# cmavro/GNN-RAG

Measured on AMD Instinct MI355X. Metric: kg_edges_aggregated_per_sec, higher is better.
Workload: dtype f32

## Files before the change

gnn-rag_amd/csrc/tables_b3.hip:

```cpp
#include "gnnrag_common.h"
#include "dense_internal.h"

namespace gnnrag {

#ifndef GNNRAG_TAB_TPW
#define GNNRAG_TAB_TPW 3
#endif
#ifndef GNNRAG_TAB_MINBLK
#define GNNRAG_TAB_MINBLK 2
#endif
constexpr int kTabTPW = GNNRAG_TAB_TPW;
constexpr int kTabNTH = 7;
constexpr int kTabNKB = 7;
constexpr int kTabSlots = 26;
constexpr int kTabQBytes = 160 * 1024 - 3 * kTabNTH * 16 * kTabSlots * 16 - 64;

struct TabArgs {
  const float* T[2];
  const float* ins;
  const float* W;
  float* P;
  const int2* rows;
  int32_t M, D, I, ldw;
  int32_t ct0;
  int32_t npass;
};

__device__ __forceinline__ int opaque_i(int x) {
  asm volatile("" : "+v"(x));
  return x;
}

template <int CTRL, int BANK>
__device__ __forceinline__ float dpp_b3(float old, float x) {
  return __int_as_float(__builtin_amdgcn_update_dpp(__float_as_int(old), __float_as_int(x), CTRL, 0xf, BANK, false));
}
__device__ __forceinline__ float row16_sum4_b3(const float (&v)[4], int lane) {
  const bool b0 = lane & 1, b1 = lane & 2;
  float w2[2];
#pragma unroll
  for (int j = 0; j < 2; ++j) {
    const float send = b0 ? v[j] : v[j + 2];
    w2[j] = (b0 ? v[j + 2] : v[j]) + dpp_b3<0xB1, 0xf>(send, send);
  }
  const float send = b1 ? w2[0] : w2[1];
  float w = (b1 ? w2[1] : w2[0]) + dpp_b3<0x4E, 0xf>(send, send);
  const float t4 = dpp_b3<0x104, 0x5>(w, w);
  w += dpp_b3<0x114, 0xA>(t4, w);
  w += dpp_b3<0x128, 0xf>(w, w);
  return w;
}

__device__ __forceinline__ int tab_lds_row(int j) {
  if (j < 64) return ((j & 3) << 4) + (j >> 2);
  return j;
}

__device__ __forceinline__ constexpr int tab_stage_rows(int ctn) { return ctn < kTabNTH ? ctn * 16 + 1 : ctn * 16; }

template <int CTN, bool QLDS>
__device__ __forceinline__ void tables_b3_part(const TabArgs& a, unsigned char* lds, int col0, int bmin, int nq) {
  constexpr int RB = kTabSlots * 16;
  constexpr int PL = kTabNTH * 16 * RB;
  constexpr int ctn = CTN;
  const int tid = threadIdx.x, lane = tid & 63, wave = tid >> 6;
  const int fr = lane & 15, fg = lane >> 4;
  const int d = blockIdx.y;
  const int D = a.D, I = a.I;
  const int ncol = min(ctn * 16, D - col0);
  const float* T = a.T[d];
  float* P = a.P + (size_t)d * a.M * D;
  const f32x4 zero4 = {0.f, 0.f, 0.f, 0.f};
  constexpr int NKB = kTabNKB;
  const int KC = D >> 2;

  const long long U = ((long long)a.M + 15) >> 4;
  const int c0 = (int)(U * blockIdx.x / gridDim.x), c1 = (int)(U * (blockIdx.x + 1) / gridDim.x);
  const int nchunk = c1 - c0;
  const int w0 = c0 + (int)((long long)nchunk * wave / 8), w1 = c0 + (int)((long long)nchunk * (wave + 1) / 8);

  if (tid < 16) reinterpret_cast<unsigned*>(lds + 3 * PL)[tid] = 0u;
  float* qarea = reinterpret_cast<float*>(lds + 3 * PL + 64);
  constexpr bool q_in_lds = QLDS;
  if (q_in_lds) {
    const float* src = a.ins + (size_t)bmin * I * D;
    for (int x = tid * 4; x < nq * I * D; x += 512 * 4)
      *reinterpret_cast<f32x4*>(qarea + x) = *reinterpret_cast<const f32x4*>(src + x);
  }

  for (int pass = 0; pass < a.npass; ++pass) {
    const int tbase = w0 + pass * kTabTPW;
    const int ntile = max(0, min(kTabTPW, w1 - tbase));
    f32x4 acc[kTabTPW][CTN];
#pragma unroll
    for (int j = 0; j < kTabTPW; ++j)
#pragma unroll
      for (int nt = 0; nt < CTN; ++nt) acc[j][nt] = zero4;

    for (int i = 0; i < I; ++i) {
      __syncthreads();
      {
        const int wcol = (1 + 2 * i + d) * D;
        const int total = tab_stage_rows(ctn) * kTabSlots * 2;
        constexpr int UN = 6;
        for (int base = 0; base < total; base += 512 * UN) {
          f32x4 v[UN];
          int off[UN];
#pragma unroll
          for (int u = 0; u < UN; ++u) {
            const int idx = base + u * 512 + tid;
            const int j = idx / (kTabSlots * 2), kc = idx - j * (kTabSlots * 2);
            v[u] = zero4;
            off[u] = idx < total ? tab_lds_row(j) * RB + kc * 8 : -1;
            if (idx < total && j < ncol && kc < KC)
              v[u] = *reinterpret_cast<const f32x4*>(a.W + (size_t)(col0 + j) * a.ldw + wcol + 4 * kc);
          }
#pragma unroll
          for (int u = 0; u < UN; ++u) {
            if (off[u] >= 0) {
              const Split3 sp = split3(v[u]);
              unsigned char* dst = lds + off[u];
              *reinterpret_cast<uint2*>(dst) = sp.hi;
              *reinterpret_cast<uint2*>(dst + PL) = sp.mid;
              *reinterpret_cast<uint2*>(dst + 2 * PL) = sp.lo;
            }
          }
        }
      }
      __syncthreads();

      int toff[kTabTPW], qoff[kTabTPW];
#pragma unroll
      for (int j = 0; j < kTabTPW; ++j) {
        const int m = min((tbase + (j < ntile ? j : 0)) * 16 + fr, a.M - 1);
        const int2 br = a.rows[m];
        toff[j] = br.y * D + 8 * fg;
        qoff[j] = ((br.x - bmin) * I + i) * D + 8 * fg;
      }
      const int kmax = D - 8;
      f32x4 traw[kTabTPW][2];
#pragma unroll
      for (int j = 0; j < kTabTPW; ++j) {
        const float* tp = T + toff[j] + (min(8 * fg, kmax) - 8 * fg);
        traw[j][0] = *reinterpret_cast<const f32x4*>(tp);
        traw[j][1] = *reinterpret_cast<const f32x4*>(tp + 4);
      }
      for (int kb = 0; kb < NKB; ++kb) {
        const bool kok = 32 * kb + 8 * fg <= kmax;
        const int kbn = min(kb + 1, NKB - 1);
        const int kon = min(32 * kbn + 8 * fg, kmax) - 8 * fg;
        const int koq = min(32 * kb + 8 * fg, kmax) - 8 * fg;
        const unsigned char* wb = lds + fr * RB + kb * 64 + fg * 16;
#pragma unroll
        for (int j = 0; j < kTabTPW; ++j) {
          if (j < ntile) {
            const f32x4 t0 = traw[j][0], t1 = traw[j][1];
            {
              const float* tp = T + toff[j] + kon;
              traw[j][0] = *reinterpret_cast<const f32x4*>(tp);
              traw[j][1] = *reinterpret_cast<const f32x4*>(tp + 4);
            }
            __builtin_amdgcn_sched_barrier(0);
            f32x4 q0, q1;
            if constexpr (QLDS) {
              const float* qp = qarea + qoff[j] + koq;
              q0 = *reinterpret_cast<const f32x4*>(qp);
              q1 = *reinterpret_cast<const f32x4*>(qp + 4);
            } else {
              const float* qp = a.ins + (size_t)bmin * I * D + qoff[j] + koq;
              q0 = *reinterpret_cast<const f32x4*>(qp);
              q1 = *reinterpret_cast<const f32x4*>(qp + 4);
            }
            const Split3 s0 = split3(kok ? __builtin_elementwise_max(t0 * q0, zero4) : zero4);
            const Split3 s1 = split3(kok ? __builtin_elementwise_max(t1 * q1, zero4) : zero4);
            typedef unsigned u32x4 __attribute__((ext_vector_type(4)));
            bf16x8 ap[3];
            ap[0] = __builtin_bit_cast(bf16x8, (u32x4){s0.hi.x, s0.hi.y, s1.hi.x, s1.hi.y});
            ap[1] = __builtin_bit_cast(bf16x8, (u32x4){s0.mid.x, s0.mid.y, s1.mid.x, s1.mid.y});
            ap[2] = __builtin_bit_cast(bf16x8, (u32x4){s0.lo.x, s0.lo.y, s1.lo.x, s1.lo.y});
            constexpr int PA[6] = {1, 2, 0, 1, 0, 0};
            constexpr int PB[6] = {1, 0, 2, 0, 1, 0};
#pragma unroll
            for (int nt = 0; nt < CTN; nt += 2) {
              bf16x8 b0[3], b1[3];
#pragma unroll
              for (int pl = 0; pl < 3; ++pl) {
                b0[pl] = __builtin_bit_cast(bf16x8, *reinterpret_cast<const f32x4*>(wb + pl * PL + nt * 16 * RB));
                b1[pl] = b0[pl];
                if (nt + 1 < CTN)
                  b1[pl] = __builtin_bit_cast(bf16x8, *reinterpret_cast<const f32x4*>(wb + pl * PL + (nt + 1) * 16 * RB));
              }
#pragma unroll
              for (int p = 0; p < 6; ++p) {
                acc[j][nt] = __builtin_amdgcn_mfma_f32_16x16x32_bf16(ap[PA[p]], b0[PB[p]], acc[j][nt], 0, 0, 0);
                if (nt + 1 < CTN)
                  acc[j][nt + 1] = __builtin_amdgcn_mfma_f32_16x16x32_bf16(ap[PA[p]], b1[PB[p]], acc[j][nt + 1], 0, 0, 0);
              }
            }
          }
        }
      }
    }

#pragma unroll
    for (int j = 0; j < kTabTPW; ++j) {
      if (j < ntile) {
        const int rbase = (tbase + j) * 16 + 4 * fg;
#pragma unroll
        for (int q = 0; q < 4; ++q) {
          const int row = rbase + q;
          if (row < a.M) {
            float* prow = P + (size_t)row * D + col0;
            static_assert(CTN >= 4, "a column part holds at least the interleaved group");
            {
              const f32x4 v = {acc[j][0][q], acc[j][1][q], acc[j][2][q], acc[j][3][q]};
              const int c = 4 * fr;
              if (c + 4 <= ncol) *reinterpret_cast<f32x4*>(prow + c) = v;
              else {
#pragma unroll
                for (int e = 0; e < 4; ++e)
                  if (c + e < ncol) prow[c + e] = v[e];
              }
            }
#pragma unroll
            for (int nt = 4; nt < CTN; ++nt) {
              const int c = nt * 16 + fr;
              if (c < ncol) prow[c] = acc[j][nt][q];
            }
          }
        }
      }
    }
  }
}

__global__ __launch_bounds__(512, GNNRAG_TAB_MINBLK) void k_tables_b3(TabArgs a) {
  extern __shared__ __attribute__((aligned(16))) unsigned char lds[];
  const int NT = (a.D + 15) >> 4;
  const int h = blockIdx.z;
  const int ctn = h == 0 ? a.ct0 : NT - a.ct0;
  const int col0 = h == 0 ? 0 : a.ct0 * 16;
  const long long U = ((long long)a.M + 15) >> 4;
  const int c0 = (int)(U * blockIdx.x / gridDim.x), c1 = (int)(U * (blockIdx.x + 1) / gridDim.x);
  const int rlo = min(c0 * 16, a.M - 1), rhi = min(c1 * 16, a.M) - 1;
  const int bmin = a.rows[rlo].x, bmax = a.rows[max(rhi, rlo)].x;
  const int nq = bmax - bmin + 1;
  const bool q_in_lds = (size_t)nq * a.I * a.D * sizeof(float) <= kTabQBytes;
#define GNNRAG_TAB_CASE(N)                                                  \
  case N:                                                                   \
    if (q_in_lds) tables_b3_part<N, true>(a, lds, col0, bmin, nq);          \
    else tables_b3_part<N, false>(a, lds, col0, bmin, nq);                  \
    break;
  switch (ctn) {
    GNNRAG_TAB_CASE(6) GNNRAG_TAB_CASE(7)
    default: break;
  }
#undef GNNRAG_TAB_CASE
}

constexpr int kVqHalf = 32 * kTabNKB;
constexpr int kVqRowB = 2 * kVqHalf * 2;
#ifndef GNNRAG_VQ_TPW
#define GNNRAG_VQ_TPW 5
#endif
#ifndef GNNRAG_VQ_UN
#define GNNRAG_VQ_UN 3
#endif
constexpr int kVqTPW = GNNRAG_VQ_TPW;

struct VqArgs {
  const unsigned char* planes;
  const float* ins;
  const float* W;
  float* P;
  const int2* rows;
  const int* rel_off;
  int32_t M, D, I, ldw, R1;
  int32_t ct0;
  int32_t nchunk;
  int32_t dir0;
  float* zero;
  int64_t zero_n;
};

template <int CTN, int UN>
__device__ __forceinline__ void vq_stage(const VqArgs& a, unsigned char* lds, const float* qarea, int col0, int ncol,
                                         int d, int s) {
  constexpr int RB = kTabSlots * 16;
  constexpr int PL = kTabNTH * 16 * RB;
  const int tid = threadIdx.x;
  const int D = a.D, I = a.I, KC = D >> 2;
  const f32x4 zero4 = {0.f, 0.f, 0.f, 0.f};
  const int total = tab_stage_rows(CTN) * kTabSlots * 2;
  for (int base = 0; base < total; base += 512 * UN) {
    f32x4 v[UN];
#pragma unroll
    for (int u = 0; u < UN; ++u) v[u] = zero4;
    for (int i = 0; i < I; ++i) {
      f32x4 w[UN];
      const float* wsrc = a.W + (size_t)col0 * a.ldw + (1 + 2 * i + d) * D;
#pragma unroll
      for (int u = 0; u < UN; ++u) {
        const int idx = base + u * 512 + tid;
        const int j = idx / (kTabSlots * 2), kc = idx - j * (kTabSlots * 2);
        w[u] = *reinterpret_cast<const f32x4*>(wsrc + (size_t)min(j, ncol - 1) * a.ldw + 4 * min(kc, KC - 1));
      }
#pragma unroll
      for (int u = 0; u < UN; ++u) {
        const int idx = base + u * 512 + tid;
        const int kc = idx % (kTabSlots * 2);
        f32x4 q = *reinterpret_cast<const f32x4*>(qarea + i * D + 4 * min(kc, KC - 1));
        q = __builtin_elementwise_max(s ? -q : q, zero4);
        v[u] += w[u] * q;
      }
    }
#pragma unroll
    for (int u = 0; u < UN; ++u) {
      const int idx = base + u * 512 + tid;
      const int j = idx / (kTabSlots * 2), kc = idx - j * (kTabSlots * 2);
      if (idx < total) {
        const Split3 sp = split3(j < ncol && kc < KC ? v[u] : zero4);
        unsigned char* dst = lds + tab_lds_row(j) * RB + kc * 8;
        *reinterpret_cast<uint2*>(dst) = sp.hi;
        *reinterpret_cast<uint2*>(dst + PL) = sp.mid;
        *reinterpret_cast<uint2*>(dst + 2 * PL) = sp.lo;
      }
    }
  }
}

template <int CTN>
__device__ __forceinline__ void tables_vq_part(const VqArgs& a, unsigned char* lds, int col0) {
  constexpr int RB = kTabSlots * 16;
  constexpr int PL = kTabNTH * 16 * RB;
  constexpr int NKB = kTabNKB;
  const int tid = threadIdx.x, lane = tid & 63, wave = tid >> 6;
  const int fr = lane & 15, fg = lane >> 4;
  const int d = a.dir0 + blockIdx.y;
  const int g = blockIdx.x / a.nchunk, ch = blockIdx.x - g * a.nchunk;
  const int D = a.D, I = a.I;
  const int r0 = a.rel_off[g], r1 = a.rel_off[g + 1];
  if (r1 <= r0) return;
  const int ncol = min(CTN * 16, D - col0);
  const int KC = D >> 2;
  const f32x4 zero4 = {0.f, 0.f, 0.f, 0.f};
  float* P = a.P + (size_t)d * a.M * D;
  const unsigned char* planes = a.planes + (size_t)d * 3 * a.R1 * kVqRowB;
  const size_t plane_stride = (size_t)a.R1 * kVqRowB;

  const int U = (r1 - r0 + 15) >> 4;
  const int c0 = U * ch / a.nchunk, c1 = U * (ch + 1) / a.nchunk;
  const int wv = __builtin_amdgcn_readfirstlane(wave);
  const int w0 = c0 + (c1 - c0) * wv / 8, w1 = c0 + (c1 - c0) * (wv + 1) / 8;
  const int npass = ((c1 - c0 + 7) / 8 + kVqTPW - 1) / kVqTPW;

  if (tid < 16) reinterpret_cast<unsigned*>(lds + 3 * PL)[tid] = 0u;
  float* qarea = reinterpret_cast<float*>(lds + 3 * PL + 64);
  for (int x = tid * 4; x < I * D; x += 512 * 4)
    *reinterpret_cast<f32x4*>(qarea + x) = *reinterpret_cast<const f32x4*>(a.ins + (size_t)g * I * D + x);

  for (int pass = 0; pass < npass; ++pass) {
    const int tbase = w0 + pass * kVqTPW;
    const int ntile = max(0, min(kVqTPW, w1 - tbase));
    f32x4 acc[kVqTPW][CTN];
#pragma unroll
    for (int j = 0; j < kVqTPW; ++j)
#pragma unroll
      for (int nt = 0; nt < CTN; ++nt) acc[j][nt] = zero4;
    unsigned aoff[kVqTPW];
#pragma unroll
    for (int j = 0; j < kVqTPW; ++j) {
      const int m = min(r0 + (tbase + (j < ntile ? j : 0)) * 16 + fr, r1 - 1);
      aoff[j] = (unsigned)a.rows[m].y * (unsigned)kVqRowB + (unsigned)fg * 16u;
    }
    const unsigned char* const plane_base[3] = {planes, planes + plane_stride, planes + 2 * plane_stride};

    for (int s = 0; s < 2; ++s) {
      __syncthreads();
      vq_stage<CTN, GNNRAG_VQ_UN>(a, lds, qarea, col0, ncol, d, s);
      __syncthreads();

      bf16x8 ap[kVqTPW][3];
#pragma unroll
      for (int j = 0; j < kVqTPW; ++j)
#pragma unroll
        for (int pl = 0; pl < 3; ++pl)
          ap[j][pl] = __builtin_bit_cast(bf16x8, *reinterpret_cast<const f32x4*>(plane_base[pl] + (aoff[j] + (unsigned)(s * (kVqHalf * 2)))));
      for (int kb = 0; kb < NKB; ++kb) {
        const int kbn = min(kb + 1, NKB - 1);
        const unsigned char* wb = lds + fr * RB + kb * 64 + fg * 16;
        constexpr int PA[6] = {1, 2, 0, 1, 0, 0};
        constexpr int PB[6] = {1, 0, 2, 0, 1, 0};
#pragma unroll
        for (int j = 0; j < kVqTPW; ++j) {
          if (j < ntile) {
#pragma unroll
            for (int nt = 0; nt < CTN; nt += 2) {
              bf16x8 b0[3], b1[3];
#pragma unroll
              for (int pl = 0; pl < 3; ++pl) {
                b0[pl] = __builtin_bit_cast(bf16x8, *reinterpret_cast<const f32x4*>(wb + pl * PL + nt * 16 * RB));
                b1[pl] = b0[pl];
                if (nt + 1 < CTN)
                  b1[pl] = __builtin_bit_cast(bf16x8, *reinterpret_cast<const f32x4*>(wb + pl * PL + (nt + 1) * 16 * RB));
              }
#pragma unroll
              for (int p = 0; p < 6; ++p) {
                acc[j][nt] = __builtin_amdgcn_mfma_f32_16x16x32_bf16(ap[j][PA[p]], b0[PB[p]], acc[j][nt], 0, 0, 0);
                if (nt + 1 < CTN)
                  acc[j][nt + 1] = __builtin_amdgcn_mfma_f32_16x16x32_bf16(ap[j][PA[p]], b1[PB[p]], acc[j][nt + 1], 0, 0, 0);
              }
            }
          }
#pragma unroll
          for (int pl = 0; pl < 3; ++pl)
            ap[j][pl] = __builtin_bit_cast(bf16x8, *reinterpret_cast<const f32x4*>(plane_base[pl] + (aoff[j] + (unsigned)(s * (kVqHalf * 2) + kbn * 64))));
        }
      }
    }

#pragma unroll
    for (int j = 0; j < kVqTPW; ++j) {
      if (j < ntile) {
        const int rbase = r0 + (tbase + j) * 16 + 4 * fg;
#pragma unroll
        for (int q = 0; q < 4; ++q) {
          const int row = rbase + q;
          if (row < r1) {
            float* prow = P + (size_t)row * D + col0;
            static_assert(CTN >= 4, "a column part holds at least the interleaved group");
            {
              const f32x4 v = {acc[j][0][q], acc[j][1][q], acc[j][2][q], acc[j][3][q]};
              const int c = 4 * fr;
              if (c + 4 <= ncol) *reinterpret_cast<f32x4*>(prow + c) = v;
              else {
#pragma unroll
                for (int e = 0; e < 4; ++e)
                  if (c + e < ncol) prow[c + e] = v[e];
              }
            }
#pragma unroll
            for (int nt = 4; nt < CTN; ++nt) {
              const int c = nt * 16 + fr;
              if (c < ncol) prow[c] = acc[j][nt][q];
            }
          }
        }
      }
    }
  }
}

__global__ __launch_bounds__(512, 2) void k_tables_vq(VqArgs a) {
  extern __shared__ __attribute__((aligned(16))) unsigned char lds[];
  if (a.zero) {
    const int64_t nb = (int64_t)gridDim.x * gridDim.y * gridDim.z;
    const int64_t lin = blockIdx.x + (int64_t)gridDim.x * (blockIdx.y + (int64_t)gridDim.y * blockIdx.z);
    for (int64_t i = lin * 512 + threadIdx.x; i < a.zero_n; i += nb * 512) a.zero[i] = 0.f;
  }
  const int NT = (a.D + 15) >> 4;
  const int h = blockIdx.z;
  const int ctn = h == 0 ? a.ct0 : NT - a.ct0;
  const int col0 = h == 0 ? 0 : a.ct0 * 16;
  switch (ctn) {
    case 6: tables_vq_part<6>(a, lds, col0); break;
    case 7: tables_vq_part<7>(a, lds, col0); break;
    default: break;
  }
}

struct UpdB3Args {
  const float* A;
  const float* W;
  const float* bias;
  const float* add;
  const float* w_s;
  const float* b_s;
  const float* mask;
  float* C;
  float* score;
  const uint8_t* add_flag;
  int32_t M, D, ldw, ct0;
};

template <int CTN, bool FL>
__device__ __forceinline__ void update_b3_part(const UpdB3Args& a, unsigned char* lds, int col0, bool first_part,
                                               int chunk, int nchunks) {
  constexpr int RB = kTabSlots * 16;
  constexpr int PL = kTabNTH * 16 * RB;
  constexpr int NKB = kTabNKB;
  const int tid = threadIdx.x, lane = tid & 63, wave = tid >> 6;
  const int fr = lane & 15, fg = lane >> 4;
  const int D = a.D;
  const int ncol = min(CTN * 16, D - col0);
  const int KC = D >> 2;
  const f32x4 zero4 = {0.f, 0.f, 0.f, 0.f};
  float* Bl = reinterpret_cast<float*>(lds + 3 * PL + 64);
  float* Sl = Bl + kTabNTH * 16;

  if (tid < 16) reinterpret_cast<unsigned*>(lds + 3 * PL)[tid] = 0u;
  for (int j = tid; j < kTabNTH * 16; j += 512) {
    Bl[j] = (j < ncol && a.bias) ? a.bias[col0 + j] : 0.f;
    Sl[j] = j < ncol ? a.w_s[col0 + j] : 0.f;
  }
  {
    const int total = tab_stage_rows(CTN) * kTabSlots * 2;
    constexpr int UN = 6;
    for (int base = 0; base < total; base += 512 * UN) {
      f32x4 v[UN];
      int off[UN];
#pragma unroll
      for (int u = 0; u < UN; ++u) {
        const int idx = base + u * 512 + tid;
        const int j = idx / (kTabSlots * 2), kc = idx - j * (kTabSlots * 2);
        v[u] = zero4;
        off[u] = idx < total ? tab_lds_row(j) * RB + kc * 8 : -1;
        if (idx < total && j < ncol && kc < KC)
          v[u] = *reinterpret_cast<const f32x4*>(a.W + (size_t)(col0 + j) * a.ldw + 4 * kc);
      }
#pragma unroll
      for (int u = 0; u < UN; ++u) {
        if (off[u] >= 0) {
          const Split3 sp = split3(v[u]);
          unsigned char* dst = lds + off[u];
          *reinterpret_cast<uint2*>(dst) = sp.hi;
          *reinterpret_cast<uint2*>(dst + PL) = sp.mid;
          *reinterpret_cast<uint2*>(dst + 2 * PL) = sp.lo;
        }
      }
    }
  }
  const long long U = ((long long)a.M + 15) >> 4;
  const int c0 = (int)(U * chunk / nchunks), c1 = (int)(U * (chunk + 1) / nchunks);
  const int nch = c1 - c0;
  int t = c0 + (int)((long long)nch * wave / 8);
  const int tend = c0 + (int)((long long)nch * (wave + 1) / 8);
  const int kmax = D - 8;
  const unsigned char* Ab = reinterpret_cast<const unsigned char*>(a.A);
  const unsigned char* addb = reinterpret_cast<const unsigned char*>(a.add);
  unsigned char* Cb = reinterpret_cast<unsigned char*>(a.C);
  const unsigned rowB = (unsigned)D * 4u;
  const unsigned k6B = (unsigned)min(32 * (NKB - 1) + 8 * fg, kmax) * 4u;
  auto a_rowoff = [&](int tile) -> unsigned { return (unsigned)min(tile * 16 + fr, a.M - 1) * rowB; };
  auto a_piece = [&](unsigned rowoff, int kb, int half) -> f32x4 {
    const unsigned off = kb < NKB - 1 ? rowoff + 32u * (unsigned)fg + (unsigned)(128 * kb + 16 * half)
                                      : rowoff + k6B + (unsigned)(16 * half);
    return *reinterpret_cast<const f32x4*>(Ab + off);
  };
  f32x4 ra[NKB][2];
  if (t < tend) {
    const unsigned ro = a_rowoff(t);
#pragma unroll
    for (int kb = 0; kb < NKB; ++kb) {
      ra[kb][0] = a_piece(ro, kb, 0);
      ra[kb][1] = a_piece(ro, kb, 1);
    }
  }
  const float bs = a.b_s[0];
  const unsigned cgB = (unsigned)(col0 + min(4 * fr, ncol - 4)) * 4u;
  unsigned ctB[CTN > 4 ? CTN - 4 : 1];
#pragma unroll
  for (int nt = 4; nt < CTN; ++nt) ctB[nt - 4] = (unsigned)(col0 + min(nt * 16 + fr, ncol - 1)) * 4u;
  unsigned fl_next = 0x01010101u;
  if (FL && t < tend) fl_next = *reinterpret_cast<const unsigned*>(a.add_flag + (size_t)t * 16 + 4 * fg);
  __syncthreads();

  for (; t < tend; ++t) {
    const int rbase = t * 16 + 4 * fg;
    const unsigned fl = fl_next;
    if (FL) fl_next = *reinterpret_cast<const unsigned*>(a.add_flag + (size_t)(t + 1 < tend ? t + 1 : t) * 16 + 4 * fg);
    f32x4 addg[4];
    float addt[CTN > 4 ? CTN - 4 : 1][4];
#pragma unroll
    for (int q = 0; q < 4; ++q) {
      int row = min(rbase + q, a.M - 1);
      if (FL && ((fl >> (8 * q)) & 0xffu) == 0u) row = a.M;
      const unsigned ro = (unsigned)row * rowB;
      addg[q] = *reinterpret_cast<const f32x4*>(addb + (ro + cgB));
#pragma unroll
      for (int nt = 4; nt < CTN; ++nt) addt[nt - 4][q] = *reinterpret_cast<const float*>(addb + (ro + ctB[nt - 4]));
    }
    float mrow = 0.f;
    {
      const int srow = min(rbase + (2 * (fr & 1) + ((fr >> 1) & 1)), a.M - 1);
      mrow = a.mask[srow];
    }
    __builtin_amdgcn_sched_barrier(0);
    f32x4 acc[CTN];
#pragma unroll
    for (int nt = 0; nt < CTN; ++nt) acc[nt] = zero4;
    const unsigned ro_next = a_rowoff(t + 1 < tend ? t + 1 : t);
    const unsigned char* wbp[3];
#pragma unroll
    for (int pl = 0; pl < 3; ++pl) {
      unsigned o = (unsigned)(fr * RB + fg * 16 + pl * PL);
      asm volatile("" : "+v"(o));
      wbp[pl] = lds + o;
    }
    constexpr int PA[6] = {1, 2, 0, 1, 0, 0};
    constexpr int PB[6] = {1, 0, 2, 0, 1, 0};
#pragma unroll
    for (int kb = 0; kb < NKB; ++kb) {
      typedef unsigned u32x4 __attribute__((ext_vector_type(4)));
      bf16x8 ap[3];
      const bool kok = kb < NKB - 1 || 32 * kb + 8 * fg <= kmax;
      const Split3 s0 = split3(kok ? ra[kb][0] : zero4);
      const Split3 s1 = split3(kok ? ra[kb][1] : zero4);
      ap[0] = __builtin_bit_cast(bf16x8, (u32x4){s0.hi.x, s0.hi.y, s1.hi.x, s1.hi.y});
      ap[1] = __builtin_bit_cast(bf16x8, (u32x4){s0.mid.x, s0.mid.y, s1.mid.x, s1.mid.y});
      ap[2] = __builtin_bit_cast(bf16x8, (u32x4){s0.lo.x, s0.lo.y, s1.lo.x, s1.lo.y});
      ra[kb][0] = a_piece(ro_next, kb, 0);
      ra[kb][1] = a_piece(ro_next, kb, 1);
#pragma unroll
      for (int nt = 0; nt < CTN; nt += 2) {
        bf16x8 b0[3], b1[3];
#pragma unroll
        for (int pl = 0; pl < 3; ++pl) {
          b0[pl] = __builtin_bit_cast(bf16x8, *reinterpret_cast<const f32x4*>(wbp[pl] + (nt * 16 * RB + kb * 64)));
          b1[pl] = b0[pl];
          if (nt + 1 < CTN)
            b1[pl] = __builtin_bit_cast(bf16x8, *reinterpret_cast<const f32x4*>(wbp[pl] + ((nt + 1) * 16 * RB + kb * 64)));
        }
#pragma unroll
        for (int p = 0; p < 6; ++p) {
          acc[nt] = __builtin_amdgcn_mfma_f32_16x16x32_bf16(ap[PA[p]], b0[PB[p]], acc[nt], 0, 0, 0);
          if (nt + 1 < CTN)
            acc[nt + 1] = __builtin_amdgcn_mfma_f32_16x16x32_bf16(ap[PA[p]], b1[PB[p]], acc[nt + 1], 0, 0, 0);
        }
      }
    }
    float part[4] = {0.f, 0.f, 0.f, 0.f};
    const f32x4 bias_g = *reinterpret_cast<const f32x4*>(Bl + min(4 * fr, kTabNTH * 16 - 4));
    const f32x4 ws_g = *reinterpret_cast<const f32x4*>(Sl + min(4 * fr, kTabNTH * 16 - 4));
#pragma unroll
    for (int q = 0; q < 4; ++q) {
      const int row = rbase + q;
      const unsigned ro = (unsigned)min(row, a.M - 1) * rowB;
      f32x4 v = {acc[0][q], acc[1][q], acc[2][q], acc[3][q]};
      v = __builtin_elementwise_max((v + bias_g) + addg[q], zero4);
      const int c = 4 * fr;
      if (c + 4 > ncol) {
        v = zero4;
      } else if (row < a.M) {
        *reinterpret_cast<f32x4*>(Cb + (ro + cgB)) = v;
      }
      part[q] += v[0] * ws_g[0] + v[1] * ws_g[1] + v[2] * ws_g[2] + v[3] * ws_g[3];
#pragma unroll
      for (int nt = 4; nt < CTN; ++nt) {
        const int cc = nt * 16 + fr;
        float x = fmaxf((acc[nt][q] + Bl[cc]) + addt[nt - 4][q], 0.f);
        if (cc >= ncol) x = 0.f;
        else if (row < a.M) *reinterpret_cast<float*>(Cb + (ro + ctB[nt - 4])) = x;
        part[q] += x * Sl[cc];
      }
    }
    {
      const float tot = row16_sum4_b3(part, lane);
      const int srow = rbase + (2 * (fr & 1) + ((fr >> 1) & 1));
      if (fr < 4 && srow < a.M) {
        const float share = first_part ? (tot + bs) + (1.0f - mrow) * kVeryNeg : tot;
        atomicAdd(a.score + srow, share);
      }
    }
  }
}

template <bool FL>
__global__ __launch_bounds__(512, 2) void k_update_b3(UpdB3Args a, int nchunks) {
  extern __shared__ __attribute__((aligned(16))) unsigned char lds[];
  const int blk = blockIdx.x;
  const int NT = (a.D + 15) >> 4;
  const int h = (blk >> 3) & 1;
  const int chunk = (blk >> 4) * 8 + (blk & 7);
  if (chunk >= nchunks) return;
  if (h == 0) update_b3_part<kTabNTH, FL>(a, lds, 0, true, chunk, nchunks);
  else if (NT - a.ct0 == 6) update_b3_part<6, FL>(a, lds, a.ct0 * 16, false, chunk, nchunks);
}

int update_b3_launch(const float* h, const float* nbr, const float* W, const float* b, const float* w_s, const float* b_s,
                     const float* mask, float* h_out, float* score, int64_t BN, int32_t D, int32_t ldw,
                     hipStream_t stream) {
  return update_b3_launch_z(h, nbr, W, b, w_s, b_s, mask, h_out, score, BN, D, ldw, stream, false);
}

int update_b3_launch_z(const float* h, const float* nbr, const float* W, const float* b, const float* w_s,
                       const float* b_s, const float* mask, float* h_out, float* score, int64_t BN, int32_t D,
                       int32_t ldw, hipStream_t stream, bool score_zeroed) {
  return update_b3_launch_f(h, nbr, nullptr, W, b, w_s, b_s, mask, h_out, score, BN, D, ldw, stream, score_zeroed);
}

bool update_b3_shape_ok(int64_t BN, int32_t D, int32_t ldw) {
  return !(D % 8 || (D + 31) / 32 != kTabNKB || (D + 15) / 16 != 13 || BN < 8192 || (BN + 1) * D * 4 >= ((int64_t)1 << 32) || ldw % 4);
}

int update_b3_launch_f(const float* h, const float* nbr, const uint8_t* add_flag, const float* W, const float* b,
                       const float* w_s, const float* b_s, const float* mask, float* h_out, float* score, int64_t BN,
                       int32_t D, int32_t ldw, hipStream_t stream, bool score_zeroed) {
  if (!update_b3_shape_ok(BN, D, ldw)) return GNNRAG_E_UNSUPPORTED;
  if ((((uintptr_t)h | (uintptr_t)nbr | (uintptr_t)W | (uintptr_t)h_out) & 15) != 0) return GNNRAG_E_UNSUPPORTED;
  UpdB3Args a;
  memset(&a, 0, sizeof(a));
  a.A = h; a.W = W; a.bias = b; a.add = nbr; a.w_s = w_s; a.b_s = b_s; a.mask = mask; a.C = h_out; a.score = score;
  a.M = (int32_t)BN; a.D = D; a.ldw = ldw; a.ct0 = kTabNTH;
  a.add_flag = add_flag;
  if (add_flag && ((uintptr_t)add_flag & 3)) return GNNRAG_E_UNSUPPORTED;
  int cus = 0;
  {
    const int rc = device_cu_count(&cus);
    if (rc) return rc;
  }
  const long long U = (BN + 15) / 16;
  int chunks = cus / 2;
  if (chunks < 1) chunks = 1;
  if ((long long)chunks * 8 > U) chunks = (int)((U + 7) / 8);
  if (!score_zeroed) GNNRAG_HIP(hipMemsetAsync(score, 0, (size_t)BN * sizeof(float), stream));
  static DeviceMask cap, cap_f;
  {
    const int rc = add_flag ? raise_lds_cap(k_update_b3<true>, cap_f) : raise_lds_cap(k_update_b3<false>, cap);
    if (rc) return rc;
  }
  const int nblk = ((chunks + 7) / 8) * 16;
  if (add_flag) hipLaunchKernelGGL(k_update_b3<true>, dim3(nblk), dim3(512), 160 * 1024, stream, a, chunks);
  else hipLaunchKernelGGL(k_update_b3<false>, dim3(nblk), dim3(512), 160 * 1024, stream, a, chunks);
  GNNRAG_LAUNCH_CHECK();
  return 0;
}

size_t tables_vq_planes_bytes(int64_t R1) { return (size_t)2 * 3 * R1 * kVqRowB; }

bool tables_vq_shape_ok(int32_t D, int32_t I) {
  return D % 8 == 0 && (D + 31) / 32 == kTabNKB && (D + 15) / 16 == 13 && I >= 1 &&
         (size_t)I * D * sizeof(float) <= (size_t)kTabQBytes;
}

int tables_vq_launch(const gnnrag_csr* csr, const void* planes, const float* ins, const float* W, float* P, int32_t D,
                     int32_t I, int32_t only_dir, hipStream_t stream) {
  return tables_vq_launch_z(csr, planes, ins, W, P, D, I, only_dir, nullptr, 0, stream);
}

int tables_vq_launch_z(const gnnrag_csr* csr, const void* planes, const float* ins, const float* W, float* P, int32_t D,
                       int32_t I, int32_t only_dir, float* zero, int64_t zero_n, hipStream_t stream) {
  if (!tables_vq_shape_ok(D, I) || csr->rel_total < 1024 || only_dir > 1) return GNNRAG_E_UNSUPPORTED;
  if ((((uintptr_t)planes | (uintptr_t)ins | (uintptr_t)W | (uintptr_t)P) & 15) != 0) return GNNRAG_E_UNSUPPORTED;
  VqArgs a;
  memset(&a, 0, sizeof(a));
  a.planes = (const unsigned char*)planes; a.ins = ins; a.W = W; a.P = P;
  a.rows = (const int2*)csr->rel_rows; a.rel_off = csr->rel_off;
  a.M = csr->rel_total; a.D = D; a.I = I; a.ldw = (2 * I + 1) * D; a.R1 = csr->R1;
  const int NT = (D + 15) / 16;
  a.ct0 = (NT + 1) / 2;
  int cus = 0;
  {
    const int rc = device_cu_count(&cus);
    if (rc) return rc;
  }
  const int ndir = only_dir < 0 ? 2 : 1;
  a.dir0 = only_dir < 0 ? 0 : only_dir;
  int nchunk = cus / (csr->B * 2 * ndir);
  const int tiles_max = (csr->rel_max + 15) / 16;
  if (nchunk > tiles_max / 8) nchunk = tiles_max / 8;
  if (nchunk < 1) nchunk = 1;
  a.nchunk = nchunk;
  a.zero = zero;
  a.zero_n = zero ? zero_n : 0;
  static DeviceMask cap;
  {
    const int rc = raise_lds_cap(k_tables_vq, cap);
    if (rc) return rc;
  }
  hipLaunchKernelGGL(k_tables_vq, dim3(csr->B * nchunk, ndir, 2), dim3(512), 160 * 1024, stream, a);
  GNNRAG_LAUNCH_CHECK();
  return 0;
}

int tables_b3_launch(const gnnrag_csr* csr, const float* T_fwd, const float* T_inv, const float* ins, const float* W,
                     float* P, int32_t D, int32_t I, hipStream_t stream) {
  if (D % 8 || (D + 31) / 32 != kTabNKB || (D + 15) / 16 != 13 || csr->rel_total < 1024) return GNNRAG_E_UNSUPPORTED;
  if ((((uintptr_t)T_fwd | (uintptr_t)T_inv | (uintptr_t)ins | (uintptr_t)W | (uintptr_t)P) & 15) != 0)
    return GNNRAG_E_UNSUPPORTED;
  TabArgs a;
  memset(&a, 0, sizeof(a));
  a.T[0] = T_fwd; a.T[1] = T_inv; a.ins = ins; a.W = W; a.P = P;
  a.rows = (const int2*)csr->rel_rows;
  a.M = csr->rel_total; a.D = D; a.I = I; a.ldw = (2 * I + 1) * D;
  const int NT = (D + 15) / 16;
  a.ct0 = NT <= kTabNTH ? NT : (NT + 1) / 2;
  const int parts = NT <= kTabNTH ? 1 : 2;
  int cus = 0;
  {
    const int rc = device_cu_count(&cus);
    if (rc) return rc;
  }
  const long long U = ((long long)a.M + 15) / 16;
  int chunks = cus / (2 * parts);
  if (chunks < 1) chunks = 1;
  if ((long long)chunks * 8 > U) chunks = (int)((U + 7) / 8);
  const int tiles_per_wave = (int)((((U + chunks - 1) / chunks) + 7) / 8);
  a.npass = (tiles_per_wave + kTabTPW - 1) / kTabTPW;
  const size_t lds = 160 * 1024;
  static DeviceMask cap;
  {
    const int rc = raise_lds_cap(k_tables_b3, cap);
    if (rc) return rc;
  }
  hipLaunchKernelGGL(k_tables_b3, dim3(chunks, 2, parts), dim3(512), lds, stream, a);
  GNNRAG_LAUNCH_CHECK();
  return 0;
}

}

extern "C" int gnnrag_relation_tables_planes(const gnnrag_csr* csr, const void* planes, const float* ins, const float* W,
                                             float* P, int32_t D, int32_t I, gnnrag_stream_t stream) {
  if (!csr || !planes || !ins || !W || !P || D <= 0 || I <= 0 || csr->rel_total < 0) return GNNRAG_E_BADARG;
  if (csr->rel_total == 0) return 0;
  return gnnrag::tables_vq_launch(csr, planes, ins, W, P, D, I, -1, (hipStream_t)stream);
}
```

Baseline: 3.015 billion.

## Use sparse SMFMAC to merge positive and negative halves of VQ products

The VQ path now builds the positive- and negative-part weight tables together, interleaved in LDS, and runs the A operand through 2:4 structured-sparse smfmac instructions. The exclusive positive/negative plane pairs are OR-compressed into one operand with a generated sparsity index. This halves the K-direction MFMA work, replacing two stage/sync passes over 7 k-blocks with three smaller stages. The cost is extra LDS writes, index computation per A load, and reliance on each 4-element group having at most two nonzeros. The stage unroll also drops from 3 to 2.

```diff
diff --git a/gnn-rag_amd/csrc/tables_b3.hip b/gnn-rag_amd/csrc/tables_b3.hip
--- a/gnn-rag_amd/csrc/tables_b3.hip
+++ b/gnn-rag_amd/csrc/tables_b3.hip
@@ -264,7 +264,7 @@
 #define GNNRAG_VQ_TPW 5
 #endif
 #ifndef GNNRAG_VQ_UN
-#define GNNRAG_VQ_UN 3
+#define GNNRAG_VQ_UN 2
 #endif
 constexpr int kVqTPW = GNNRAG_VQ_TPW;
 
@@ -283,50 +283,98 @@
   int64_t zero_n;
 };
 
+typedef __bf16 bf16x16 __attribute__((ext_vector_type(16)));
+constexpr int kVqSub = 3 * 64;
+
+__device__ __forceinline__ uint4 vq_interleave(uint2 p, uint2 n) {
+  return make_uint4((p.x & 0xffffu) | (n.x << 16), (p.x >> 16) | (n.x & 0xffff0000u), (p.y & 0xffffu) | (n.y << 16),
+                    (p.y >> 16) | (n.y & 0xffff0000u));
+}
+__device__ __forceinline__ bf16x16 vq_read_b(const unsigned char* p) {
+  struct { f32x4 lo, hi; } v = {*reinterpret_cast<const f32x4*>(p), *reinterpret_cast<const f32x4*>(p + kVqSub)};
+  return __builtin_bit_cast(bf16x16, v);
+}
+
+__device__ __forceinline__ int vq_row(int x, int nb) { return nb == 3 ? (int)(((unsigned)x * 43691u) >> 17) : x; }
+
 template <int CTN, int UN>
 __device__ __forceinline__ void vq_stage(const VqArgs& a, unsigned char* lds, const float* qarea, int col0, int ncol,
-                                         int d, int s) {
+                                         int d, int blk0, int nb) {
   constexpr int RB = kTabSlots * 16;
   constexpr int PL = kTabNTH * 16 * RB;
+  const int total = CTN * 16 * 8 * nb;
   const int tid = threadIdx.x;
   const int D = a.D, I = a.I, KC = D >> 2;
   const f32x4 zero4 = {0.f, 0.f, 0.f, 0.f};
-  const int total = tab_stage_rows(CTN) * kTabSlots * 2;
   for (int base = 0; base < total; base += 512 * UN) {
-    f32x4 v[UN];
-#pragma unroll
-    for (int u = 0; u < UN; ++u) v[u] = zero4;
+    f32x4 vp[UN], vn[UN];
+#pragma unroll
+    for (int u = 0; u < UN; ++u) vp[u] = vn[u] = zero4;
     for (int i = 0; i < I; ++i) {
       f32x4 w[UN];
       const float* wsrc = a.W + (size_t)col0 * a.ldw + (1 + 2 * i + d) * D;
 #pragma unroll
       for (int u = 0; u < UN; ++u) {
         const int idx = base + u * 512 + tid;
-        const int j = idx / (kTabSlots * 2), kc = idx - j * (kTabSlots * 2);
+        const int j = vq_row(idx >> 3, nb), kc = (blk0 + (idx >> 3) - j * nb) * 8 + (idx & 7);
         w[u] = *reinterpret_cast<const f32x4*>(wsrc + (size_t)min(j, ncol - 1) * a.ldw + 4 * min(kc, KC - 1));
       }
 #pragma unroll
       for (int u = 0; u < UN; ++u) {
         const int idx = base + u * 512 + tid;
-        const int kc = idx % (kTabSlots * 2);
-        f32x4 q = *reinterpret_cast<const f32x4*>(qarea + i * D + 4 * min(kc, KC - 1));
-        q = __builtin_elementwise_max(s ? -q : q, zero4);
-        v[u] += w[u] * q;
+        const int kc = (blk0 + (idx >> 3) - vq_row(idx >> 3, nb) * nb) * 8 + (idx & 7);
+        const f32x4 q = *reinterpret_cast<const f32x4*>(qarea + i * D + 4 * min(kc, KC - 1));
+        vp[u] += w[u] * __builtin_elementwise_max(q, zero4);
+        vn[u] += w[u] * __builtin_elementwise_max(-q, zero4);
       }
     }
 #pragma unroll
     for (int u = 0; u < UN; ++u) {
       const int idx = base + u * 512 + tid;
-      const int j = idx / (kTabSlots * 2), kc = idx - j * (kTabSlots * 2);
+      const int j = vq_row(idx >> 3, nb), b = (idx >> 3) - j * nb, pc = idx & 7, kc = (blk0 + b) * 8 + pc;
       if (idx < total) {
-        const Split3 sp = split3(j < ncol && kc < KC ? v[u] : zero4);
-        unsigned char* dst = lds + tab_lds_row(j) * RB + kc * 8;
-        *reinterpret_cast<uint2*>(dst) = sp.hi;
-        *reinterpret_cast<uint2*>(dst + PL) = sp.mid;
-        *reinterpret_cast<uint2*>(dst + 2 * PL) = sp.lo;
-      }
-    }
-  }
+        const bool live = j < ncol && kc < KC;
+        const Split3 sp = split3(live ? vp[u] : zero4), sn = split3(live ? vn[u] : zero4);
+        unsigned char* dst = lds + tab_lds_row(j) * RB + (pc >> 2) * kVqSub + b * 64 + (pc & 3) * 16;
+        *reinterpret_cast<uint4*>(dst) = vq_interleave(sp.hi, sn.hi);
+        *reinterpret_cast<uint4*>(dst + PL) = vq_interleave(sp.mid, sn.mid);
+        *reinterpret_cast<uint4*>(dst + 2 * PL) = vq_interleave(sp.lo, sn.lo);
+      }
+    }
+  }
+}
+
+struct VqA {
+  bf16x8 pl[3];
+  int idx;
+};
+struct VqRaw {
+  uint4 p[3], n[3];
+};
+__device__ __forceinline__ VqRaw vq_load_a(const unsigned char* const (&plane_base)[3], unsigned off) {
+  VqRaw r;
+#pragma unroll
+  for (int pl = 0; pl < 3; ++pl) {
+    r.p[pl] = *reinterpret_cast<const uint4*>(plane_base[pl] + off);
+    r.n[pl] = *reinterpret_cast<const uint4*>(plane_base[pl] + (off + (unsigned)(kVqHalf * 2)));
+  }
+  return r;
+}
+__device__ __forceinline__ VqA vq_compress(const VqRaw& r) {
+  VqA o;
+#pragma unroll
+  for (int pl = 0; pl < 3; ++pl) {
+    const uint4 c = make_uint4(r.p[pl].x | r.n[pl].x, r.p[pl].y | r.n[pl].y, r.p[pl].z | r.n[pl].z, r.p[pl].w | r.n[pl].w);
+    o.pl[pl] = __builtin_bit_cast(bf16x8, c);
+  }
+  const unsigned m[4] = {r.n[0].x | r.n[1].x | r.n[2].x, r.n[0].y | r.n[1].y | r.n[2].y, r.n[0].z | r.n[1].z | r.n[2].z,
+                         r.n[0].w | r.n[1].w | r.n[2].w};
+  unsigned ix = 0x8888u;
+#pragma unroll
+  for (int i = 0; i < 4; ++i)
+    ix |= (min(m[i] & 0xffffu, 1u) | (min(m[i] >> 16, 1u) << 2)) << (4 * i);
+  o.idx = (int)ix;
+  return o;
 }
 
 template <int CTN>
@@ -334,6 +382,7 @@
   constexpr int RB = kTabSlots * 16;
   constexpr int PL = kTabNTH * 16 * RB;
   constexpr int NKB = kTabNKB;
+  constexpr int NPAIR = (kVqTPW + 1) / 2;
   const int tid = threadIdx.x, lane = tid & 63, wave = tid >> 6;
   const int fr = lane & 15, fg = lane >> 4;
   const int d = a.dir0 + blockIdx.y;
@@ -342,7 +391,6 @@
   const int r0 = a.rel_off[g], r1 = a.rel_off[g + 1];
   if (r1 <= r0) return;
   const int ncol = min(CTN * 16, D - col0);
-  const int KC = D >> 2;
   const f32x4 zero4 = {0.f, 0.f, 0.f, 0.f};
   float* P = a.P + (size_t)d * a.M * D;
   const unsigned char* planes = a.planes + (size_t)d * 3 * a.R1 * kVqRowB;
@@ -354,7 +402,6 @@
   const int w0 = c0 + (c1 - c0) * wv / 8, w1 = c0 + (c1 - c0) * (wv + 1) / 8;
   const int npass = ((c1 - c0 + 7) / 8 + kVqTPW - 1) / kVqTPW;
 
-  if (tid < 16) reinterpret_cast<unsigned*>(lds + 3 * PL)[tid] = 0u;
   float* qarea = reinterpret_cast<float*>(lds + 3 * PL + 64);
   for (int x = tid * 4; x < I * D; x += 512 * 4)
     *reinterpret_cast<f32x4*>(qarea + x) = *reinterpret_cast<const f32x4*>(a.ins + (size_t)g * I * D + x);
@@ -375,46 +422,48 @@
     }
     const unsigned char* const plane_base[3] = {planes, planes + plane_stride, planes + 2 * plane_stride};
 
-    for (int s = 0; s < 2; ++s) {
+    for (int s = 0; s < 3; ++s) {
       __syncthreads();
-      vq_stage<CTN, GNNRAG_VQ_UN>(a, lds, qarea, col0, ncol, d, s);
+      const int nblk = s < 2 ? 3 : 1;
+      vq_stage<CTN, GNNRAG_VQ_UN>(a, lds, qarea, col0, ncol, d, 3 * s, nblk);
       __syncthreads();
-
-      bf16x8 ap[kVqTPW][3];
-#pragma unroll
-      for (int j = 0; j < kVqTPW; ++j)
-#pragma unroll
-        for (int pl = 0; pl < 3; ++pl)
-          ap[j][pl] = __builtin_bit_cast(bf16x8, *reinterpret_cast<const f32x4*>(plane_base[pl] + (aoff[j] + (unsigned)(s * (kVqHalf * 2)))));
-      for (int kb = 0; kb < NKB; ++kb) {
-        const int kbn = min(kb + 1, NKB - 1);
+      for (int kb = 0; kb < nblk; ++kb) {
+        const int blk = 3 * s + kb;
         const unsigned char* wb = lds + fr * RB + kb * 64 + fg * 16;
         constexpr int PA[6] = {1, 2, 0, 1, 0, 0};
         constexpr int PB[6] = {1, 0, 2, 0, 1, 0};
 #pragma unroll
-        for (int j = 0; j < kVqTPW; ++j) {
-          if (j < ntile) {
-#pragma unroll
-            for (int nt = 0; nt < CTN; nt += 2) {
-              bf16x8 b0[3], b1[3];
-#pragma unroll
-              for (int pl = 0; pl < 3; ++pl) {
-                b0[pl] = __builtin_bit_cast(bf16x8, *reinterpret_cast<const f32x4*>(wb + pl * PL + nt * 16 * RB));
-                b1[pl] = b0[pl];
-                if (nt + 1 < CTN)
-                  b1[pl] = __builtin_bit_cast(bf16x8, *reinterpret_cast<const f32x4*>(wb + pl * PL + (nt + 1) * 16 * RB));
+        for (int p = 0; p < NPAIR; ++p) {
+          const int j0 = 2 * p, j1 = 2 * p + 1 < kVqTPW ? 2 * p + 1 : 2 * p;
+          const bool two = 2 * p + 1 < kVqTPW;
+          VqA cur[2];
+          {
+            cur[0] = vq_compress(vq_load_a(plane_base, aoff[j0] + (unsigned)(blk * 64)));
+            cur[1] = two ? vq_compress(vq_load_a(plane_base, aoff[j1] + (unsigned)(blk * 64))) : cur[0];
+          }
+          if (two && j0 < ntile) {
+#pragma unroll
+            for (int nt = 0; nt < CTN; ++nt) {
+              bf16x16 b[3];
+#pragma unroll
+              for (int pl = 0; pl < 3; ++pl) b[pl] = vq_read_b(wb + pl * PL + nt * 16 * RB);
+#pragma unroll
+              for (int q = 0; q < 6; ++q) {
+                acc[j0][nt] = __builtin_amdgcn_smfmac_f32_16x16x64_bf16(cur[0].pl[PA[q]], b[PB[q]], acc[j0][nt], cur[0].idx, 0, 0);
+                acc[j1][nt] = __builtin_amdgcn_smfmac_f32_16x16x64_bf16(cur[1].pl[PA[q]], b[PB[q]], acc[j1][nt], cur[1].idx, 0, 0);
               }
-#pragma unroll
-              for (int p = 0; p < 6; ++p) {
-                acc[j][nt] = __builtin_amdgcn_mfma_f32_16x16x32_bf16(ap[j][PA[p]], b0[PB[p]], acc[j][nt], 0, 0, 0);
-                if (nt + 1 < CTN)
-                  acc[j][nt + 1] = __builtin_amdgcn_mfma_f32_16x16x32_bf16(ap[j][PA[p]], b1[PB[p]], acc[j][nt + 1], 0, 0, 0);
-              }
+            }
+          } else if (!two && j0 < ntile) {
+#pragma unroll
+            for (int nt = 0; nt < CTN; ++nt) {
+              bf16x16 b[3];
+#pragma unroll
+              for (int pl = 0; pl < 3; ++pl) b[pl] = vq_read_b(wb + pl * PL + nt * 16 * RB);
+#pragma unroll
+              for (int q = 0; q < 6; ++q)
+                acc[j0][nt] = __builtin_amdgcn_smfmac_f32_16x16x64_bf16(cur[0].pl[PA[q]], b[PB[q]], acc[j0][nt], cur[0].idx, 0, 0);
             }
           }
-#pragma unroll
-          for (int pl = 0; pl < 3; ++pl)
-            ap[j][pl] = __builtin_bit_cast(bf16x8, *reinterpret_cast<const f32x4*>(plane_base[pl] + (aoff[j] + (unsigned)(s * (kVqHalf * 2) + kbn * 64))));
         }
       }
     }
```

New measurement: 3.046 billion, median of 6. +1.0%, better.
